# bjing2016/mdgen

Hardware: AMD Instinct MI355X
Metric: sampled MD frames/sec (higher is better)
Workload: dtype bf16

## Files before the change

mdgen_amd/build.py:

```python
from __future__ import annotations

import argparse
import concurrent.futures as cf
import os
import shutil
import subprocess

HERE = os.path.dirname(os.path.abspath(__file__))
CSRC = os.path.join(HERE, "csrc")
OBJ = os.path.join(HERE, "build")
LIB = os.path.join(HERE, "libmdgen_amd.so")
SOURCES = ["api.hip", "k_gemm.hip", "k_rows.hip", "k_flash.hip", "k_small.hip", "k_se3.hip", "k_fp32.hip", "k_optim.hip", "k_fp32_bwd.hip", "k_attn16.hip", "k_wide16.hip", "k_ode.hip"]
HEADERS = ["common.h", "dev.h", "panel.h", "rows.h", "linear.h", "kernels.h", "train.inc", "ode.inc", os.path.join("..", "..", "include", "mdgen_amd.h")]
FLAGS = ["--offload-arch=gfx950", "-O3", "-std=c++17", "-fPIC", "-fno-gpu-rdc", "-fno-slp-vectorize", "-Wall",
         "-Wno-unused-function", "-Wno-pass-failed"]
EXTRA = {"k_flash.hip": ["-fno-honor-nans"]}


def flags_for(src: str):
    return FLAGS + EXTRA.get(os.path.basename(src), [])


def hipcc() -> str:
    for c in (os.environ.get("HIPCC"), shutil.which("hipcc"), "/opt/rocm/bin/hipcc"):
        if c and os.path.exists(c):
            return c
    raise RuntimeError("hipcc not found (set HIPCC)")


_MFMA_RE = None


def check_isa(cc: str, src: str) -> None:
    import re
    import tempfile
    with tempfile.TemporaryDirectory() as td:
        out = os.path.join(td, "k.s")
        r = subprocess.run([cc] + [f for f in flags_for(src) if f not in ("-fPIC",)] + ["-S", "--cuda-device-only", src, "-o", out],
                           capture_output=True, text=True)
        if r.returncode != 0:
            raise RuntimeError("ISA check failed to compile " + src + "\n" + r.stderr)
        pat = re.compile(r"v_mfma_\w+ ([va])\[(\d+):(\d+)\], ([va])\[(\d+):(\d+)\], ([va])\[(\d+):(\d+)\], (.*)$")
        n = 0
        own_m0 = os.path.basename(src) in ("k_rows.hip", "k_wide16.hip")
        in_asm = False
        for line in open(out):
            if own_m0:
                if "#ASMSTART" in line:
                    in_asm = True
                elif "#ASMEND" in line:
                    in_asm = False
                elif not in_asm and re.search(r"\bm0\b", line.split(";")[0]):
                    raise RuntimeError(f"{os.path.basename(src)}: compiler-generated M0 access: {line.strip()}")
            if re.search(r"\bv_pk_(mul|add|fma)_f32\b", line):
                raise RuntimeError(f"{os.path.basename(src)}: packed fp32 VALU op emitted: {line.strip()}")
            m = pat.search(line)
            if not m:
                continue
            n += 1
            g = m.groups()
            dc, ac, bc = g[0], g[3], g[6]
            d0, d1, a0, a1, b0, b1 = int(g[1]), int(g[2]), int(g[4]), int(g[5]), int(g[7]), int(g[8])
            if (ac == dc and not (a1 < d0 or a0 > d1)) or (bc == dc and not (b1 < d0 or b0 > d1)):
                raise RuntimeError(f"{os.path.basename(src)}: MFMA destination overlaps a source operand: {line.strip()}")
    return n


def _stale(target, deps):
    if not os.path.exists(target):
        return True
    t = os.path.getmtime(target)
    return any(os.path.getmtime(d) > t for d in deps)


def build(force: bool = False, jobs: int = 8, verbose: bool = True) -> str:
    os.makedirs(OBJ, exist_ok=True)
    cc = hipcc()
    hdrs = [os.path.join(CSRC, h) for h in HEADERS]
    todo = []
    objs = []
    for src in SOURCES:
        s = os.path.join(CSRC, src)
        o = os.path.join(OBJ, src.replace(".hip", ".o"))
        objs.append(o)
        if force or _stale(o, [s] + hdrs):
            todo.append((s, o))

    def compile_one(so):
        s, o = so
        cmd = [cc] + flags_for(s) + ["-c", s, "-o", o]
        r = subprocess.run(cmd, capture_output=True, text=True)
        if r.returncode != 0:
            raise RuntimeError("hipcc failed: " + " ".join(cmd) + "\n" + r.stdout + r.stderr)
        if os.path.basename(s).startswith("k_"):
            try:
                check_isa(cc, s)
            except Exception:
                if os.path.exists(o):
                    os.remove(o)
                raise
        return s, r.stderr

    if todo:
        with cf.ThreadPoolExecutor(max_workers=jobs) as ex:
            for s, err in ex.map(compile_one, todo):
                if verbose:
                    print("compiled", os.path.basename(s))
                    if err.strip():
                        print(err.strip())
    if force or todo or _stale(LIB, objs):
        cmd = [cc, "--offload-arch=gfx950", "-shared", "-fPIC", "-o", LIB] + objs
        r = subprocess.run(cmd, capture_output=True, text=True)
        if r.returncode != 0:
            raise RuntimeError("link failed: " + " ".join(cmd) + "\n" + r.stdout + r.stderr)
        if verbose:
            print("linked", LIB)
    return LIB


if __name__ == "__main__":
    ap = argparse.ArgumentParser()
    ap.add_argument("--force", action="store_true")
    ap.add_argument("-j", type=int, default=8)
    a = ap.parse_args()
    print(build(force=a.force, jobs=a.j))
```

mdgen_amd/csrc/k_flash.hip:

```cpp
#include "kernels.h"
#include "panel.h"
#include <type_traits>

namespace mdg {

__device__ __forceinline__ bf16x8 frag16(const unsigned char* p) { return *reinterpret_cast<const bf16x8*>(p); }

__device__ __forceinline__ bf16x8 frag8(const unsigned char* p) {
    const u32x2 v = *reinterpret_cast<const u32x2*>(p);
    const u32x4 w = u32x4{v[0], v[1], 0u, 0u};
    return __builtin_bit_cast(bf16x8, w);
}

struct KTile {
    u32x4 k0;
    u32x4 k1;
};
struct VTile {
    u32x4 v0;
    u32x4 v1;
};
struct QTile {
    bf16x8 q0, q1;
};
struct PTile {
    u32x4 p0, p1;
};

struct Half {
    f32x16 o;
    float m;
    unsigned long long unanch;
};

__device__ __forceinline__ float half_max(float x) {
    const auto r = __builtin_amdgcn_permlane32_swap(__float_as_uint(x), __float_as_uint(x), false, false);
    return fmaxf(__uint_as_float(r[0]), __uint_as_float(r[1]));
}

__device__ __forceinline__ float round_bf16(float x) { return __uint_as_float(pack_bf16(x, 0.f) << 16); }

__device__ __forceinline__ float set_shift(QTile& q, float m, int hh) {
    const float hi = round_bf16(m), lo = round_bf16(m - hi);
    if (hh == 0) {
        q.q1[4] = (__bf16)(-hi);
        q.q1[5] = (__bf16)(-lo);
    }
    return hi + lo;
}

constexpr float kAnchor = 63.f;

__device__ __forceinline__ void mask_scores(f32x16& s, uint32_t vm, int hh) {
    uint32_t vmh;
    asm volatile("v_lshrrev_b32 %0, %1, %2" : "=v"(vmh) : "v"(4 * hh), "s"(vm));
#pragma unroll
    for (int r = 0; r < 16; ++r) {
        const bool ok = (vmh >> ((r & 3) + 8 * (r >> 2))) & 1u;
        s[r] = ok ? s[r] : -1e30f;
    }
}

__device__ __forceinline__ f32x16 scores(const KTile& k, const QTile& q) {
    const bf16x8 k0 = __builtin_bit_cast(bf16x8, k.k0), k1 = __builtin_bit_cast(bf16x8, k.k1);
    const f32x16 zero = {0.f, 0.f, 0.f, 0.f, 0.f, 0.f, 0.f, 0.f, 0.f, 0.f, 0.f, 0.f, 0.f, 0.f, 0.f, 0.f};
    f32x16 s = __builtin_amdgcn_mfma_f32_32x32x16_bf16(k0, q.q0, zero, 0, 0, 0);
    s = __builtin_amdgcn_mfma_f32_32x32x16_bf16(k1, q.q1, s, 0, 0, 0);
    asm volatile("" :: "v"(k0), "v"(k1), "v"(q.q0), "v"(q.q1));
    return s;
}

__device__ __forceinline__ void block(const KTile& kn, const QTile& qn, f32x16& n,
                                      const VTile& vp, const PTile& pp, f32x16& od,
                                      const f32x16& s, PTile& pc) {
    const bf16x8 k0 = __builtin_bit_cast(bf16x8, kn.k0), k1 = __builtin_bit_cast(bf16x8, kn.k1);
    const f32x16 zero = {0.f, 0.f, 0.f, 0.f, 0.f, 0.f, 0.f, 0.f, 0.f, 0.f, 0.f, 0.f, 0.f, 0.f, 0.f, 0.f};
    od = __builtin_amdgcn_mfma_f32_32x32x16_bf16(__builtin_bit_cast(bf16x8, vp.v0), __builtin_bit_cast(bf16x8, pp.p0), od, 0, 0, 0);
    n = __builtin_amdgcn_mfma_f32_32x32x16_bf16(k0, qn.q0, zero, 0, 0, 0);
    od = __builtin_amdgcn_mfma_f32_32x32x16_bf16(__builtin_bit_cast(bf16x8, vp.v1), __builtin_bit_cast(bf16x8, pp.p1), od, 0, 0, 0);
    n = __builtin_amdgcn_mfma_f32_32x32x16_bf16(k1, qn.q1, n, 0, 0, 0);
    float e[16];
#pragma unroll
    for (int j = 0; j < 16; ++j) e[j] = __builtin_amdgcn_exp2f(s[j]);
#pragma unroll
    for (int j = 0; j < 4; ++j) {
#ifdef MDGEN_DEV_FLASH_TRUNC
        pc.p0[j] = __builtin_amdgcn_perm(__float_as_uint(e[2 * j + 1]), __float_as_uint(e[2 * j]), 0x07060302u);
        pc.p1[j] = __builtin_amdgcn_perm(__float_as_uint(e[9 + 2 * j]), __float_as_uint(e[8 + 2 * j]), 0x07060302u);
#else
        pc.p0[j] = pack_bf16(e[2 * j], e[2 * j + 1]);
        pc.p1[j] = pack_bf16(e[8 + 2 * j], e[9 + 2 * j]);
#endif
    }
#pragma unroll
    for (int g = 0; g < 4; ++g) {
        __builtin_amdgcn_sched_group_barrier(0x008, 1, 0);
        __builtin_amdgcn_sched_group_barrier(0x402, 6, 0);
    }
    asm volatile("" : "+v"(pc.p0), "+v"(pc.p1) : "v"(k0), "v"(k1), "v"(qn.q0), "v"(qn.q1));
}

constexpr float kDefer = 8.f;

__device__ __forceinline__ void softmax_stats(Half& st, f32x16& s, QTile& q, uint32_t vm, int hh) {
    if (vm != 0xffffffffu) mask_scores(s, vm, hh);
    float t = fmaxf(s[0], s[1]);
#pragma unroll
    for (int r = 2; r < 16; r += 2) t = fmaxf(fmaxf(t, s[r]), s[r + 1]);
    t = half_max(t);
    if ((__builtin_amdgcn_ballot_w64(t > kDefer) | st.unanch) != 0) {
        const bool fin = t > -1e29f;
        const bool un = (st.unanch >> lane_id()) & 1ull;
        const bool mv = (t > kDefer) | (un & fin & (t < -kDefer));
        st.unanch &= ~__builtin_amdgcn_ballot_w64(fin);
        const float r = set_shift(q, mv ? st.m + t : st.m, hh);
        const float e = r - st.m;
        st.m = r;
        const float a = __builtin_amdgcn_exp2f(fminf(-e, 0.f));
#pragma unroll
        for (int i = 0; i < 16; ++i) {
            st.o[i] *= a;
            s[i] -= e;
        }
    }
}

#ifdef MDGEN_DEV_FLASH_STAMPS
__device__ unsigned long long g_flash_stamps[32768 * 16];
extern "C" int mdgen_dev_flash_stamps(void* host, size_t bytes) {
    return (int)hipMemcpyFromSymbol(host, HIP_SYMBOL(g_flash_stamps), bytes);
}
#define FLASH_STAMP(slot, v)                                                                          \
    if (lane == 0 && (long)blockIdx.x * 4 + w < 32768) g_flash_stamps[((long)blockIdx.x * 4 + w) * 16 + (slot)] = (v)
__device__ unsigned long long g_fproj_stamps[8192 * 16];
extern "C" int mdgen_dev_fproj_stamps(void* host, size_t bytes) {
    return (int)hipMemcpyFromSymbol(host, HIP_SYMBOL(g_fproj_stamps), bytes);
}
#define FPROJ_STAMP(slot, v)                                                                          \
    if (lane_id() == 0 && (long)blockIdx.x * 4 + w < 8192) g_fproj_stamps[((long)blockIdx.x * 4 + w) * 16 + (slot)] = (v)
#define FLASH_STAMP_ROW(w, hg) ((w) + 4096 * (hg))
#else
#define FLASH_STAMP(slot, v)
#define FPROJ_STAMP(slot, v)
#define FLASH_STAMP_ROW(w, hg) (w)
#endif

template <int N, class F>
__device__ __forceinline__ void static_for(F&& f) {
    if constexpr (N > 0) {
        static_for<N - 1>(f);
        f(std::integral_constant<int, N - 1>{});
    }
}

struct FlashStoreGlobal {
    __bf16* obuf;
    AxisMap ax;
    int seq, head;
    __device__ __forceinline__ void row(int, int pos, u32x2 a, u32x2 b, u32x2 c) const {
        u32x2* d = reinterpret_cast<u32x2*>(obuf + ax.token(seq, pos) * kC + head * kDH + (lane_id() >> 5) * 12);
        d[0] = a;
        d[1] = b;
        d[2] = c;
    }
    __device__ __forceinline__ void pad(int, int) const {}
};

template <int NQ>
struct FlashPre {
    QTile q[NQ];
    u32x4 kb0;
    u32x2 kb1;
    f32x4 bvl[3];
    KTile k0t;
    uint32_t vmw;
};

__device__ __forceinline__ void* flash_uniform_ptr(const unsigned char* q_) {
    const unsigned long long a = (unsigned long long)q_;
    const unsigned lo = __builtin_amdgcn_readfirstlane((unsigned)a), hi = __builtin_amdgcn_readfirstlane((unsigned)(a >> 32));
    return (void*)(((unsigned long long)hi << 32) | lo);
}

template <int NQ>
__device__ __forceinline__ void flash_prefetch(const FlashParams p, const int seq, const int head, const int qc, FlashPre<NQ>& pre) {
    const int lane = lane_id(), hh = lane >> 5;
    const int len = p.ax.len, nt = p.ax.ntile();
    const long ftile = (long)(seq * kH + head) * nt;
    const unsigned char* qb = p.qf + ftile * kFragQ;
    const int qt0 = NQ * qc;
#pragma unroll
    for (int j = 0; j < NQ; ++j) {
        const int qt = (qt0 + j) * 32 < len ? qt0 + j : qt0;
        pre.q[j].q0 = frag16(qb + (long)qt * kFragQ + lane * 16);
        pre.q[j].q1 = frag8(qb + (long)qt * kFragQ + 1024 + lane * 8);
    }
    const bool bias_alone = (len & 31) == 0 && len >= 32;
    const unsigned char* kb = p.kf + (ftile + (bias_alone ? (len >> 5) : 0)) * kFragK + hh * 32 * 16;
    pre.kb0 = *reinterpret_cast<const u32x4*>(kb);
    pre.kb1 = *reinterpret_cast<const u32x2*>(kb + 1024);
    const f32x4* bv = reinterpret_cast<const f32x4*>(p.bias_v + head * kDH + hh * 12);
    pre.bvl[0] = bv[0];
    pre.bvl[1] = bv[1];
    pre.bvl[2] = bv[2];
    const __amdgpu_buffer_rsrc_t krs = __builtin_amdgcn_make_buffer_rsrc(flash_uniform_ptr(p.kf + ftile * kFragK), 0, 0x7fffffff, 0x00020000);
    pre.k0t.k0 = __builtin_amdgcn_raw_buffer_load_b128(krs, lane * 16, 0, 0);
    pre.k0t.k1 = __builtin_amdgcn_raw_buffer_load_b128(krs, lane * 16 + 1024, 0, 0);
    pre.vmw = (p.vmask + (long)seq * p.vmask_stride)[lane];
}

template <int NQ, class Store>
__device__ __forceinline__ void flash_job(const FlashParams p, const int seq, const int head, const int qc, const int w,
                                          const FlashPre<NQ> pre, const Store store) {
    const int lane = lane_id(), hh = lane >> 5, ql = lane & 31;
    FLASH_STAMP(0, __builtin_amdgcn_s_memtime());
    FLASH_STAMP(4, __builtin_amdgcn_s_memrealtime());
    const int len = p.ax.len, nt = p.ax.ntile();
    const long ftile = (long)(seq * kH + head) * nt;
    const int qt0 = NQ * qc;
    QTile q[NQ];
    bool qvalid[NQ];
#pragma unroll
    for (int j = 0; j < NQ; ++j) {
        qvalid[j] = (qt0 + j) * 32 < len;
        q[j] = pre.q[j];
    }
    const bool bias_alone = (len & 31) == 0 && len >= 32;
    const u32x4 kb0 = pre.kb0;
    const u32x2 kb1 = pre.kb1;
    const f32x4 bvl[3] = {pre.bvl[0], pre.bvl[1], pre.bvl[2]};

    const __amdgpu_buffer_rsrc_t krs = __builtin_amdgcn_make_buffer_rsrc(flash_uniform_ptr(p.kf + ftile * kFragK), 0, 0x7fffffff, 0x00020000);
    const __amdgpu_buffer_rsrc_t vrs = __builtin_amdgcn_make_buffer_rsrc(flash_uniform_ptr(p.vf + ftile * kFragV), 0, 0x7fffffff, 0x00020000);
    const int koff = lane * 16;
    const int voff = ql <= kDH ? hh * 400 + ql * 16 : (int)0x80000000;
    auto issue_k = [&](KTile& t, int kt) __attribute__((always_inline)) {
        t.k0 = __builtin_amdgcn_raw_buffer_load_b128(krs, koff, kt * kFragK, 0);
        t.k1 = __builtin_amdgcn_raw_buffer_load_b128(krs, koff + 1024, kt * kFragK, 0);
    };
    auto issue_v = [&](VTile& t, int kt) __attribute__((always_inline)) {
        t.v0 = __builtin_amdgcn_raw_buffer_load_b128(vrs, voff, kt * kFragV, 0);
        t.v1 = __builtin_amdgcn_raw_buffer_load_b128(vrs, voff + 800, kt * kFragV, 0);
    };
    const KTile k0t = pre.k0t;
    const uint32_t* vmrow = p.vmask + (long)seq * p.vmask_stride;
    uint32_t vmw = pre.vmw;

    Half h[NQ];
    f32x16 s[2];
    PTile pt[2];
    KTile kx, ky;
    VTile vx, vy;
    int rot = 0, nrun = 1;
    auto phys = [&](int i) __attribute__((always_inline)) {
        const int t = i + rot;
        return t >= nrun ? t - nrun : t;
    };
    auto tile = [&](auto robust, int ti, KTile& kc, KTile& kn, VTile& vc, VTile& vprev) __attribute__((always_inline)) {
        constexpr bool kRobust = decltype(robust)::value;
        const int t = kRobust ? ti : phys(ti);
        const uint32_t vm = __builtin_amdgcn_readlane(vmw, t & 63);
        static_for<NQ>([&](auto J) __attribute__((always_inline)) {
            constexpr int j = decltype(J)::value;
            if constexpr (kRobust) softmax_stats(h[j], s[j & 1], q[j], vm, hh);
            else if (vm != 0xffffffffu) mask_scores(s[j & 1], vm, hh);
            __builtin_amdgcn_sched_barrier(0);
            if constexpr (j == 0) block(kc, q[1], s[1], vprev, pt[(NQ - 1) & 1], h[NQ - 1].o, s[0], pt[0]);
            else if constexpr (j < NQ - 1) block(kc, q[j + 1], s[(j + 1) & 1], vc, pt[(j - 1) & 1], h[j - 1].o, s[j & 1], pt[j & 1]);
            else block(kn, q[0], s[0], vc, pt[(j - 1) & 1], h[j - 1].o, s[j & 1], pt[j & 1]);
            __builtin_amdgcn_sched_barrier(0);
#ifndef MDGEN_DEV_FLASH_NOLOAD
            if constexpr (j == 0) issue_v(vprev, kRobust ? ti + 1 : phys(ti + 1));
            if constexpr (j == NQ - 2) issue_k(kc, kRobust ? ti + 2 : phys(ti + 2));
            if constexpr (j == 0 || j == NQ - 2) __builtin_amdgcn_sched_barrier(0);
#endif
        });
    };
    auto run = [&](auto robust, const int nt, const int rot_) __attribute__((always_inline)) {
        rot = rot_;
        nrun = nt;
#pragma unroll
        for (int j = 0; j < NQ; ++j)
#pragma unroll
            for (int r = 0; r < 16; ++r) h[j].o[r] = opaque_zero();
        pt[(NQ - 1) & 1].p0 = pt[(NQ - 1) & 1].p1 = u32x4{0u, 0u, 0u, 0u};
        if (nt > 64) vmw = vmrow[lane];
        issue_k(kx, phys(0));
        issue_v(vy, phys(0));
        issue_k(ky, phys(1));
        issue_v(vx, phys(0));
        __builtin_amdgcn_sched_barrier(0);
        s[0] = scores(kx, q[0]);
        int t = 0;
        for (; t + 1 < nt; t += 2) {
            if ((t & 63) == 0 && t) vmw = vmrow[t + lane];
            tile(robust, t, kx, ky, vx, vy);
            tile(robust, t + 1, ky, kx, vy, vx);
        }
        const bf16x8 lp0 = __builtin_bit_cast(bf16x8, pt[(NQ - 1) & 1].p0), lp1 = __builtin_bit_cast(bf16x8, pt[(NQ - 1) & 1].p1);
        if (t < nt) {
            if ((t & 63) == 0 && t) vmw = vmrow[t + lane];
            tile(robust, t, kx, ky, vx, vy);
            h[NQ - 1].o = __builtin_amdgcn_mfma_f32_32x32x16_bf16(__builtin_bit_cast(bf16x8, vx.v0), __builtin_bit_cast(bf16x8, pt[(NQ - 1) & 1].p0), h[NQ - 1].o, 0, 0, 0);
            h[NQ - 1].o = __builtin_amdgcn_mfma_f32_32x32x16_bf16(__builtin_bit_cast(bf16x8, vx.v1), __builtin_bit_cast(bf16x8, pt[(NQ - 1) & 1].p1), h[NQ - 1].o, 0, 0, 0);
        } else {
            h[NQ - 1].o = __builtin_amdgcn_mfma_f32_32x32x16_bf16(__builtin_bit_cast(bf16x8, vy.v0), lp0, h[NQ - 1].o, 0, 0, 0);
            h[NQ - 1].o = __builtin_amdgcn_mfma_f32_32x32x16_bf16(__builtin_bit_cast(bf16x8, vy.v1), lp1, h[NQ - 1].o, 0, 0, 0);
        }
    };

    if (nt <= 64 && !p.force_robust) {
        const uint32_t want = lane == (len >> 5) ? 1u << (len & 31) : 0u;
        const bool only_bias = __builtin_amdgcn_ballot_w64(lane < nt && vmw != want) == 0;
        if (only_bias) {
            const f32x4 b0 = bvl[0], b1 = bvl[1], b2 = bvl[2];
            const u32x2 d0 = {pack_bf16(b0[0], b0[1]), pack_bf16(b0[2], b0[3])}, d1 = {pack_bf16(b1[0], b1[1]), pack_bf16(b1[2], b1[3])},
                        d2 = {pack_bf16(b2[0], b2[1]), pack_bf16(b2[2], b2[3])};
#pragma unroll
            for (int j = 0; j < NQ; ++j) {
                const int pos = (qt0 + j) * 32 + ql;
                if (qvalid[j] && pos < len) store.row(j, pos, d0, d1, d2);
                else store.pad(j, pos);
            }
            return;
        }
    }
    const int nt_fast = bias_alone ? nt - 1 : nt;
    float sbias[NQ], vbias[12];
    if (bias_alone) {
        const f32x4 b0 = bvl[0], b1 = bvl[1], b2 = bvl[2];
#pragma unroll
        for (int i = 0; i < 4; ++i) {
            vbias[i] = round_bf16(b0[i]);
            vbias[4 + i] = round_bf16(b1[i]);
            vbias[8 + i] = round_bf16(b2[i]);
        }
#pragma unroll
        for (int j = 0; j < NQ; ++j) {
            const u32x4 qa = __builtin_bit_cast(u32x4, q[j].q0);
            const u32x4 qb_ = __builtin_bit_cast(u32x4, q[j].q1);
            float d = 0.f;
#pragma unroll
            for (int i = 0; i < 4; ++i) d += bf16_lo(qa[i]) * bf16_lo(kb0[i]) + bf16_hi(qa[i]) * bf16_hi(kb0[i]);
#pragma unroll
            for (int i = 0; i < 2; ++i) d += bf16_lo(qb_[i]) * bf16_lo(kb1[i]) + bf16_hi(qb_[i]) * bf16_hi(kb1[i]);
            sbias[j] = d + __shfl_xor(d, 32, 64);
        }
    }
    bool robust_needed = p.force_robust != 0;
    {
        const uint32_t vm0 = __builtin_amdgcn_readlane(vmw, 0);
#pragma unroll
        for (int j = 0; j < NQ; ++j) {
            f32x16 s0 = scores(k0t, q[j]);
            if (vm0 != 0xffffffffu) mask_scores(s0, vm0, hh);
            float t0 = fmaxf(s0[0], s0[1]);
#pragma unroll
            for (int r = 2; r < 16; r += 2) t0 = fmaxf(fmaxf(t0, s0[r]), s0[r + 1]);
            t0 = half_max(t0);
            robust_needed |= __builtin_amdgcn_ballot_w64(!(t0 > -1e29f)) != 0;
            h[j].m = set_shift(q[j], t0 + kAnchor, hh);
        }
    }
    FLASH_STAMP(1, __builtin_amdgcn_s_memtime());
    FLASH_STAMP(6, (unsigned long long)robust_needed);
    FLASH_STAMP(8, (unsigned long long)__float_as_uint(h[0].m));
    if (!robust_needed) {
        run(std::false_type{}, nt_fast, (p.rotate && nt_fast > 2 && nt <= 64) ? (qc * nt_fast) / ((len + 32 * NQ - 1) / (32 * NQ)) : 0);
        if (bias_alone) {
#pragma unroll
            for (int j = 0; j < NQ; ++j) {
                const float pb = __builtin_amdgcn_exp2f(sbias[j] - h[j].m);
#pragma unroll
                for (int r = 0; r < 12; ++r) h[j].o[r] += pb * vbias[r];
                if (hh == 0) h[j].o[12] += pb;
            }
        }
        FLASH_STAMP(2, __builtin_amdgcn_s_memtime());
        bool bad = false;
#pragma unroll
        for (int j = 0; j < NQ; ++j) {
            const uint32_t lj = __float_as_uint(h[j].o[12]);
            bad |= (lj & 0x7f800000u) == 0x7f800000u;
            bad |= hh == 0 && (lj & 0x7f800000u) == 0u;
#pragma unroll
            for (int i = 0; i < 16; ++i) bad |= (__float_as_uint(h[j].o[i]) & 0x7f800000u) == 0x7f800000u;
        }
        FLASH_STAMP(9, (unsigned long long)__builtin_amdgcn_ballot_w64(bad));
        robust_needed = __builtin_amdgcn_ballot_w64(bad) != 0;
#ifdef MDGEN_DEV_FLASH_NOFALLBACK
        robust_needed = false;
#endif
    }
    if (robust_needed) {
#pragma unroll
        for (int j = 0; j < NQ; ++j) {
            h[j].m = 0.f;
            h[j].unanch = ~0ull;
            set_shift(q[j], 0.f, hh);
        }
        run(std::true_type{}, nt, 0);
    }
    FLASH_STAMP(3, __builtin_amdgcn_s_memtime());
    FLASH_STAMP(11, (unsigned long long)__float_as_uint(h[0].m));
#ifdef MDGEN_DEV_FLASH_STAMPS
    if (lane == 0 && (long)blockIdx.x * 4 + w < 32768) g_flash_stamps[((long)blockIdx.x * 4 + w) * 16 + 6] |= (unsigned long long)robust_needed << 1;
#endif
#pragma unroll
    for (int j = 0; j < NQ; ++j) {
        const float l = __shfl(h[j].o[12], ql, 64);
        const int pos = (qt0 + j) * 32 + ql;
        if (qvalid[j] && pos < len) {
            const float inv = 1.0f / l;
            const f32x16 o = h[j].o;
            store.row(j, pos, u32x2{pack_bf16(o[0] * inv, o[1] * inv), pack_bf16(o[2] * inv, o[3] * inv)},
                      u32x2{pack_bf16(o[4] * inv, o[5] * inv), pack_bf16(o[6] * inv, o[7] * inv)},
                      u32x2{pack_bf16(o[8] * inv, o[9] * inv), pack_bf16(o[10] * inv, o[11] * inv)});
        } else {
            store.pad(j, pos);
        }
    }
    FLASH_STAMP(5, __builtin_amdgcn_s_memrealtime());
}

template <int NQ>
__global__ __launch_bounds__(256, NQ == 2 ? 3 : 2) void k_flash(const FlashParams p) {
    const int w = __builtin_amdgcn_readfirstlane(wave_id());
    const int nqc = (p.ax.len + 32 * NQ - 1) / (32 * NQ);
    const int xcd = blockIdx.x & 7, rest = blockIdx.x >> 3;
    const int qc = rest % nqc, pair = (rest / nqc) * 8 + xcd;
    const int seq = pair >> 2, hg = pair & 3;
    if (seq >= p.ax.nseq) return;
    const int head = hg * 4 + w;
    FlashPre<NQ> pre;
    flash_prefetch<NQ>(p, seq, head, qc, pre);
    flash_job<NQ>(p, seq, head, qc, w, pre, FlashStoreGlobal{p.obuf, p.ax, seq, head});
}

typedef __attribute__((address_space(3))) unsigned char lds_byte;
struct FlashStorePanel {
    lds_byte* panel;
    int head;
    __device__ __forceinline__ void put(int j, u32x2 a, u32x2 b, u32x2 c) const {
        const int lane = lane_id(), row = 32 * j + (lane & 31), byte = head * 48 + (lane >> 5) * 24;
        typedef __attribute__((address_space(3))) u32x2 lds_u32x2;
        *reinterpret_cast<lds_u32x2*>(panel + panel_off(row, byte, kC * 2)) = a;
        *reinterpret_cast<lds_u32x2*>(panel + panel_off(row, byte + 8, kC * 2)) = b;
        *reinterpret_cast<lds_u32x2*>(panel + panel_off(row, byte + 16, kC * 2)) = c;
    }
    __device__ __forceinline__ void row(int j, int, u32x2 a, u32x2 b, u32x2 c) const { put(j, a, b, c); }
    __device__ __forceinline__ void pad(int j, int) const { put(j, u32x2{0u, 0u}, u32x2{0u, 0u}, u32x2{0u, 0u}); }
};

__global__ __launch_bounds__(256, 2) void k_flash_proj(const FlashProjParams p) {
    constexpr int NQ = 2;
    static_assert(32 * NQ == kPanel, "one workgroup = one 64-row panel");
    __shared__ __attribute__((aligned(16))) unsigned char smem[sizeof(PanelRows) + kPanel * kC * 2];
    PanelRows* pr = reinterpret_cast<PanelRows*>(smem);
    unsigned char* panel = smem + sizeof(PanelRows);
    const int w = __builtin_amdgcn_readfirstlane(wave_id());
    const int nqc = (p.f.ax.len + kPanel - 1) / kPanel;
    const int xcd = blockIdx.x & 7, rest = blockIdx.x >> 3;
    const int qc = rest % nqc, seq = (rest / nqc) * 8 + xcd;
    if (seq >= p.f.ax.nseq) return;
    FPROJ_STAMP(0, __builtin_amdgcn_s_memtime());
    FPROJ_STAMP(8, __builtin_amdgcn_s_memrealtime());
    FPROJ_STAMP(10, (unsigned long long)__builtin_amdgcn_s_getreg((31 << 11) | 4));
    setup_rows_axis(pr, p.f.ax, seq, qc * kPanel, p.mm);
    FlashPre<NQ> cur;
    flash_prefetch<NQ>(p.f, seq, w, qc, cur);
#pragma unroll 1
    for (int hg = 0; hg < 4; ++hg) {
        FlashPre<NQ> nxt;
        flash_prefetch<NQ>(p.f, seq, 4 * (hg < 3 ? hg + 1 : 3) + w, qc, nxt);
        __builtin_amdgcn_sched_barrier(0);
        flash_job<NQ>(p.f, seq, 4 * hg + w, qc, FLASH_STAMP_ROW(w, hg), cur, FlashStorePanel{(lds_byte*)panel, 4 * hg + w});
        cur = nxt;
        FPROJ_STAMP(1 + hg, __builtin_amdgcn_s_memtime());
    }
    __syncthreads();
    FPROJ_STAMP(5, __builtin_amdgcn_s_memtime());
    const int lane = lane_id();
    f32x16 acc[6];
#ifndef MDGEN_DEV_FLASH_NOEARLY
    EpiPre<8> ep;
    epi_rmw_request<8>(0, 0, pr, 96 * w, p.h, ep);
    __builtin_amdgcn_sched_barrier(0);
#endif
    zero_acc<6>(acc);
    wave_gemm<2, 3, 24, false>(panel, kC * 2, 0, 0, p.wo + (size_t)(3 * w) * 24 * 64 + lane, 24 * 64, acc);
    FPROJ_STAMP(6, __builtin_amdgcn_s_memtime());
    __syncthreads();
#ifndef MDGEN_DEV_FLASH_NOEARLY
    epilogue_gate_residual_lds_pre<3>(acc, pr, reinterpret_cast<float*>(panel) + w * (32 * 96), 96 * w, p.bo, p.mm, p.gate_chunk, true,
                                      p.h, ep);
#else
    epilogue_gate_residual_lds<3>(acc, pr, reinterpret_cast<float*>(panel) + w * (32 * 96), 96 * w, p.bo, p.mm, p.gate_chunk, true,
                                  p.h);
#endif
    FPROJ_STAMP(7, __builtin_amdgcn_s_memtime());
    FPROJ_STAMP(9, __builtin_amdgcn_s_memrealtime());
}

__global__ __launch_bounds__(512, 1) void k_flash_proj8(const FlashProjParams p) {
    constexpr int NQ = 4, kRows = 32 * NQ;
    __shared__ __attribute__((aligned(16))) unsigned char smem[2 * sizeof(PanelRows) + kRows * kC * 2];
    PanelRows* pr = reinterpret_cast<PanelRows*>(smem);
// ... 77 lines not shown
```

mdgen_amd/csrc/k_gemm.hip:

```cpp
#include "kernels.h"
#include "panel.h"

namespace mdg {

constexpr int kRowB = kC * 2;
constexpr int kPanelBytes = kPanel * kRowB;

template <bool ROPE, int TT = 2>
__device__ __forceinline__ void epilogue_heads_T(const f32x16* acc , const PanelRows* pr, int w,
                                                 const float* __restrict__ bias_perm, const float* __restrict__ rope,
                                                 bool small, int pos0, int len, int seq, int ntile, int tile0,
                                                 unsigned char* __restrict__ frag, __bf16* __restrict__ small_dst,
                                                 int which) {
    const int lane = lane_id(), hh = lane >> 5, tk = lane & 31;
    f32x4 bq[4][3];
    {
        const f32x4* bp = reinterpret_cast<const f32x4*>(bias_perm + (w * 2 + hh) * 48);
#pragma unroll
        for (int hd = 0; hd < 4; ++hd)
#pragma unroll
            for (int c = 0; c < 3; ++c) bq[hd][c] = bp[hd * 3 + c];
    }
    int tokv[TT], posv[TT];
    f32x4 rq[TT][4];
#pragma unroll
    for (int tt = 0; tt < TT; ++tt) {
        const int row = tt * 32 + tk;
        tokv[tt] = pr->tok[row];
        int pos = small ? (tokv[tt] >= 0 ? tokv[tt] % len : 0) : pos0 + row;
        if (pos > len) pos = len;
        posv[tt] = pos;
        if (ROPE) {
            const f32x4* rc = reinterpret_cast<const f32x4*>(rope + (long)pos * kRopeRow + 16 * hh);
#pragma unroll
            for (int i = 0; i < 4; ++i) rq[tt][i] = rc[i];
        }
    }
#pragma unroll
    for (int tt = 0; tt < TT; ++tt) {
        const int token = tokv[tt];
        const bool valid = token >= 0;
        float cs[6], sn[6];
        if (ROPE) {
#pragma unroll
            for (int p = 0; p < 6; ++p) {
                cs[p] = rq[tt][p >> 2][p & 3];
                sn[p] = rq[tt][2 + (p >> 2)][p & 3];
            }
        }
        const int tile = tile0 + tt;
#pragma unroll
        for (int hd = 0; hd < 4; ++hd) {
            float e[12];
#pragma unroll
            for (int c = 0; c < 3; ++c) {
                const int ap = 3 * hd + c, ft = ap >> 2, a = ap & 3;
#pragma unroll
                for (int b = 0; b < 4; ++b) e[4 * c + b] = acc[ft * TT + tt][4 * a + b] + bq[hd][c][b];
            }
            if (ROPE) {
#pragma unroll
                for (int p = 0; p < 6; ++p) {
                    const float x1 = e[2 * p], x2 = e[2 * p + 1];
                    e[2 * p] = x1 * cs[p] - x2 * sn[p];
                    e[2 * p + 1] = x2 * cs[p] + x1 * sn[p];
                }
            }
            uint32_t u[6];
#pragma unroll
            for (int i = 0; i < 6; ++i) u[i] = pack_bf16(e[2 * i], e[2 * i + 1]);
            const int head = 4 * w + hd;
            if (small) {
                if (valid) {
                    u32x2* d = reinterpret_cast<u32x2*>(small_dst + (long)token * (3 * kC) + which * kC + head * kDH + hh * 12);
                    d[0] = u32x2{u[0], u[1]};
                    d[1] = u32x2{u[2], u[3]};
                    d[2] = u32x2{u[4], u[5]};
                }
            } else if (tile < ntile) {
                if (which == 1) {
                    unsigned char* base = frag + ((long)(seq * kH + head) * ntile + tile) * kFragK;
                    *reinterpret_cast<u32x4*>(base + lane * 16) = u32x4{u[0], u[1], u[2], u[3]};
                    *reinterpret_cast<u32x4*>(base + 1024 + lane * 16) = u32x4{u[4], u[5], 0x3f803f80u, 0u};
                } else {
                    unsigned char* base = frag + ((long)(seq * kH + head) * ntile + tile) * kFragQ;
                    *reinterpret_cast<u32x4*>(base + lane * 16) = u32x4{u[0], u[1], u[2], u[3]};
                    *reinterpret_cast<u32x2*>(base + 1024 + lane * 8) = u32x2{u[4], u[5]};
                }
            }
        }
    }
}

template <int TT = 2>
__device__ __forceinline__ void epilogue_v_flash(const f32x16* acc , int w,
                                                 const float* __restrict__ bias_perm, int seq, int ntile, int tile0,
                                                 unsigned char* __restrict__ vf) {
    const int lane = lane_id(), hh = lane >> 5, n = lane & 31;
#pragma unroll
    for (int j = 0; j < 3; ++j) {
        const int col = 32 * j + n;
        const int hd = col / kDH, d = col - hd * kDH;
        const float b = bias_perm[w * 96 + col];
        const int head = 4 * w + hd;
#pragma unroll
        for (int tt = 0; tt < TT; ++tt) {
            const int tile = tile0 + tt;
            if (tile < ntile) {
                unsigned char* base = vf + ((long)(seq * kH + head) * ntile + tile) * kFragV + hh * 400 + d * 16;
                const f32x16 a = acc[tt * 3 + j];
                *reinterpret_cast<u32x4*>(base) = u32x4{pack_bf16(a[0] + b, a[1] + b), pack_bf16(a[2] + b, a[3] + b),
                                                         pack_bf16(a[4] + b, a[5] + b), pack_bf16(a[6] + b, a[7] + b)};
                *reinterpret_cast<u32x4*>(base + 800) =
                    u32x4{pack_bf16(a[8] + b, a[9] + b), pack_bf16(a[10] + b, a[11] + b),
                          pack_bf16(a[12] + b, a[13] + b), pack_bf16(a[14] + b, a[15] + b)};
            }
        }
    }
    if (lane < 32) {
        const int hd = lane & 3, tt = (lane >> 2) & 1, h2 = (lane >> 3) & 1, ks = lane >> 4;
        const int tile = tile0 + tt;
        if (tt < TT && tile < ntile)
            *reinterpret_cast<u32x4*>(vf + ((long)(seq * kH + 4 * w + hd) * ntile + tile) * kFragV + ks * 800 + h2 * 400 + kDH * 16) =
                u32x4{0x3f803f80u, 0x3f803f80u, 0x3f803f80u, 0x3f803f80u};
    }
}

__device__ __forceinline__ void write_bias_slots(const QkvParams& p, int seq, int w, bool do_k = true, bool do_v = true, int tpp = 2) {
    const int lane = lane_id();
    const int len = p.ax.len, nt = p.ax.ntile();
    const int kt = len >> 5, sl = len & 31;
    if (kt >= tpp * p.panels_per_seq) {
#pragma unroll
        for (int hd = 0; hd < 4; ++hd) {
            const long ft = (long)(seq * kH + 4 * w + hd) * nt + kt;
            u32x4* kd = reinterpret_cast<u32x4*>(p.kf + ft * kFragK);
            u32x4* vd = reinterpret_cast<u32x4*>(p.vf + ft * kFragV);
            const u32x4 z = {0u, 0u, 0u, 0u}, ones = {0x3f803f80u, 0x3f803f80u, 0x3f803f80u, 0x3f803f80u};
            if (do_k) {
                kd[lane] = z;
                kd[64 + lane] = u32x4{0u, 0u, 0x3f803f80u, 0u};
            }
            const int r0 = lane, r1 = 64 + lane;
            if (do_v) {
                vd[r0] = (r0 % 25) == kDH ? ones : z;
                if (r1 < 100) vd[r1] = (r1 % 25) == kDH ? ones : z;
            }
        }
        __builtin_amdgcn_sched_barrier(0);
    }
    if (do_k && lane < 8) {
        const int hd = lane & 3, hh = lane >> 2, head = 4 * w + hd;
        const float* bk = p.bias_k + head * kDH;
        const float* rc = p.rope + (long)len * kRopeRow + 16 * hh;
        float e[12];
#pragma unroll
        for (int pp = 0; pp < 6; ++pp) {
            const int i = 6 * hh + pp;
            const float x1 = bk[i], x2 = bk[i + 12], c = rc[pp], sn = rc[8 + pp];
            e[2 * pp] = x1 * c - x2 * sn;
            e[2 * pp + 1] = x2 * c + x1 * sn;
        }
        unsigned char* base = p.kf + ((long)(seq * kH + head) * nt + kt) * kFragK;
        *reinterpret_cast<u32x4*>(base + (hh * 32 + sl) * 16) =
            u32x4{pack_bf16(e[0], e[1]), pack_bf16(e[2], e[3]), pack_bf16(e[4], e[5]), pack_bf16(e[6], e[7])};
        *reinterpret_cast<u32x4*>(base + 1024 + (hh * 32 + sl) * 16) =
            u32x4{pack_bf16(e[8], e[9]), pack_bf16(e[10], e[11]), 0x3f803f80u, 0u};
    }
    if (do_v && lane < kDH) {
        const int d = lane;
        const int dpsi = 12 * ((d >> 2) & 1) + 4 * (d >> 3) + (d & 3);
        const int hk = (sl >> 2) & 1, r = (sl & 3) + 4 * (sl >> 3);
#pragma unroll
        for (int hd = 0; hd < 4; ++hd) {
            const int head = 4 * w + hd;
            unsigned char* base = p.vf + ((long)(seq * kH + head) * nt + kt) * kFragV;
            const uint32_t v = pack_bf16(p.bias_v[head * kDH + dpsi], 0.f);
            *reinterpret_cast<uint16_t*>(base + (r >> 3) * 800 + hk * 400 + d * 16 + (r & 7) * 2) = (uint16_t)v;
        }
    }
}

#ifdef MDGEN_DEV_QKV_STAMPS
__device__ unsigned long long g_qkv_stamps[16384 * 8];
extern "C" int mdgen_dev_qkv_stamps(void* host, size_t bytes) {
    return (int)hipMemcpyFromSymbol(host, HIP_SYMBOL(g_qkv_stamps), bytes);
}
#define QKV_STAMP(slot)                                                                                      \
    if (!SMALL && lane_id() == 0 && (long)blockIdx.x * 4 + wave_id() < 16384)                                  \
    g_qkv_stamps[((long)blockIdx.x * 4 + wave_id()) * 8 + (slot)] = __builtin_amdgcn_s_memtime()
__device__ unsigned long long g_attn4_stamps[8192 * 16];
extern "C" int mdgen_dev_attn4_stamps(void* host, size_t bytes) {
    return (int)hipMemcpyFromSymbol(host, HIP_SYMBOL(g_attn4_stamps), bytes);
}
#define ATTN4_STAMP_DECL unsigned long long a4st[11] = {}
#define ATTN4_STAMP(slot)                          \
    a4st[slot] = __builtin_amdgcn_s_memtime();     \
    __builtin_amdgcn_sched_barrier(0)
#define ATTN4_STAMP_FLUSH                                                                                   \
    if (lane_id() == 0 && (long)blockIdx.x * 4 + wave_id() < 8192) {                                          \
        _Pragma("unroll") for (int k = 0; k < 11; ++k)                                                        \
            g_attn4_stamps[((long)blockIdx.x * 4 + wave_id()) * 16 + k] = a4st[k];                            \
    }
#else
#define QKV_STAMP(slot)
#define ATTN4_STAMP_DECL
#define ATTN4_STAMP(slot)
#define ATTN4_STAMP_FLUSH
#endif

template <bool SMALL, bool PRE = false>
__global__ __launch_bounds__(256, 2) void k_ln_qkv(const QkvParams p) {
    __shared__ __attribute__((aligned(16))) unsigned char smem[sizeof(PanelRows) + kPanelBytes];
    PanelRows* pr = reinterpret_cast<PanelRows*>(smem);
    unsigned char* panel = smem + sizeof(PanelRows);
    int seq = 0, pos0 = 0, tile0 = 0;
    if (SMALL) {
        setup_rows_linear(pr, (long)blockIdx.x * kPanel, p.nrows, p.mm);
    } else {
        seq = blockIdx.x / p.panels_per_seq;
        const int pn = blockIdx.x - seq * p.panels_per_seq;
        pos0 = pn * kPanel;
        tile0 = pn * 2;
        setup_rows_axis(pr, p.ax, seq, pos0, p.mm);
        if (wave_id() == 0) {
            const int lane = lane_id(), len = p.ax.len, pos = pos0 + lane;
            const float mv = p.mk.at(p.ax.token(seq, pos < len ? pos : len - 1));
            const unsigned long long bal = __ballot(pos == len || (pos < len && mv != 0.f));
            uint32_t* vm = p.vmask + (long)seq * p.vmask_stride;
            if (lane < 2) vm[tile0 + lane] = (uint32_t)(bal >> (32 * lane));
            if (pn == p.panels_per_seq - 1) {
                const int idx = tile0 + 2 + lane;
                if (idx < p.vmask_stride) vm[idx] = idx == (len >> 5) ? 1u << (len & 31) : 0u;
                if (idx + 64 < p.vmask_stride) vm[idx + 64] = 0u;
            }
        }
    }
    QKV_STAMP(0);
    __syncthreads();
    const int w = __builtin_amdgcn_readfirstlane(wave_id()), lane = lane_id();
    f32x16 acc[6];
    if (PRE) {
        prologue_bf16<kC>(panel, pr, p.obuf);
        __syncthreads();
        zero_acc<6>(acc);
        wave_gemm<2, 3, 24, false>(panel, kRowB, 0, 0, p.wo + (size_t)(3 * w) * 24 * 64 + lane, 24 * 64, acc);
        __syncthreads();
        epilogue_gate_residual_lds<3>(acc, pr, reinterpret_cast<float*>(panel) + w * (32 * 96), 96 * w, p.bo, p.mm, p.gate_chunk,
                                      true, p.h_rw);
        __syncthreads();
    }
    prologue_ln<false>(panel, pr, PRE ? p.h_rw : p.h, p.mm, p.shift_chunk, p.scale_chunk, 1e-6f);
    __syncthreads();
    QKV_STAMP(1);
    const int ntile = p.ax.ntile();
    const int len = p.ax.len;
    zero_acc<6>(acc);
    wave_gemm<2, 3, 24, true>(panel, kRowB, 0, 0, p.wq + (size_t)(3 * w) * 24 * 64 + lane, 24 * 64, acc);
    QKV_STAMP(2);
    epilogue_heads_T<true>(acc, pr, w, p.bq, p.rope, SMALL, pos0, len, seq, ntile, tile0, p.qf, p.qkv_small, 0);
    __builtin_amdgcn_sched_barrier(0);
    QKV_STAMP(3);
    zero_acc<6>(acc);
    wave_gemm<2, 3, 24, true>(panel, kRowB, 0, 0, p.wk + (size_t)(3 * w) * 24 * 64 + lane, 24 * 64, acc);
    QKV_STAMP(4);
    epilogue_heads_T<true>(acc, pr, w, p.bk, p.rope, SMALL, pos0, len, seq, ntile, tile0, p.kf, p.qkv_small, 1);
    __builtin_amdgcn_sched_barrier(0);
    QKV_STAMP(5);
    zero_acc<6>(acc);
    if (SMALL) {
        wave_gemm<2, 3, 24, true>(panel, kRowB, 0, 0, p.wv + (size_t)(3 * w) * 24 * 64 + lane, 24 * 64, acc);
        epilogue_heads_T<false>(acc, pr, w, p.bv, nullptr, true, pos0, len, seq, ntile, tile0, nullptr, p.qkv_small, 2);
    } else {
        wave_gemm<2, 3, 24, false>(panel, kRowB, 0, 0, p.wv + (size_t)(3 * w) * 24 * 64 + lane, 24 * 64, acc);
        QKV_STAMP(6);
        epilogue_v_flash(acc, w, p.bv, seq, ntile, tile0, p.vf);
        if ((int)blockIdx.x - seq * p.panels_per_seq == p.panels_per_seq - 1) {
            __builtin_amdgcn_sched_barrier(0);
            write_bias_slots(p, seq, w);
        }
        QKV_STAMP(7);
    }
}

template <int J>
__device__ __forceinline__ float quad_bcast(float v) {
    return __builtin_bit_cast(float, __builtin_amdgcn_update_dpp(0, __builtin_bit_cast(int, v), J * 0x55, 0xf, 0xf, true));
}
__device__ __forceinline__ float half_sum(float x) {
    const auto r = __builtin_amdgcn_permlane32_swap(__float_as_uint(x), __float_as_uint(x), false, false);
    return __uint_as_float(r[0]) + __uint_as_float(r[1]);
}
template <int TT = 2>
__device__ __forceinline__ void head_values(const f32x16* acc, int tt, int hd, const f32x4 (&bq)[3], float (&e)[12]) {
#pragma unroll
    for (int c = 0; c < 3; ++c) {
        const int ap = 3 * hd + c, ft = ap >> 2, a = ap & 3;
#pragma unroll
        for (int b = 0; b < 4; ++b) e[4 * c + b] = acc[ft * TT + tt][4 * a + b] + bq[c][b];
    }
}
__device__ __forceinline__ void load_head_bias(const float* bias_perm, int w, int hh, f32x4 (&bq)[4][3]) {
    const f32x4* bp = reinterpret_cast<const f32x4*>(bias_perm + (w * 2 + hh) * 48);
#pragma unroll
    for (int hd = 0; hd < 4; ++hd)
#pragma unroll
        for (int c = 0; c < 3; ++c) bq[hd][c] = bp[hd * 3 + c];
}


template <bool SPLIT, bool HALF = false>
__global__ __launch_bounds__(512, 1) void k_ln_qkv8(const QkvParams p) {
    static_assert(!HALF || SPLIT, "32-row workgroups exist in the split form only");
    constexpr int TT = HALF ? 1 : 2, kRows = 32 * TT;
    __shared__ __attribute__((aligned(16))) unsigned char smem[sizeof(PanelRows) + kPanelBytes];
    PanelRows* pr = reinterpret_cast<PanelRows*>(smem);
    unsigned char* panel = smem + sizeof(PanelRows);
    const int blk = SPLIT ? blockIdx.x >> 1 : blockIdx.x, half = SPLIT ? blockIdx.x & 1 : 0;
    const int seq = blk / p.panels_per_seq;
    const int pn = blk - seq * p.panels_per_seq;
// ... 956 lines not shown
```

Measured before the change: 120,000.

## Stop storing constant K-fragment padding; synthesize it in registers in flash attention

The K fragment's second half used to store a constant bf16 1.0 / zero pair per lane in global memory, and every K tile load read 16 bytes for it. Producers now write only the 8 meaningful bytes. The flash kernel loads 8 bytes and fills the constant lanes once with inline asm, so the compiler cannot rematerialise them, and a build check rejects any compiler-generated copy of the constant. Q prefetch also moves to buffer loads. This cuts K write and read traffic and register moves, at the cost of coupling the producer layout to the consumer and relying on the registers staying intact across the loop.

```diff
diff --git a/mdgen_amd/build.py b/mdgen_amd/build.py
--- a/mdgen_amd/build.py
+++ b/mdgen_amd/build.py
@@ -44,14 +44,16 @@
         n = 0
         own_m0 = os.path.basename(src) in ("k_rows.hip", "k_wide16.hip")
         in_asm = False
+        k_const = os.path.basename(src) == "k_flash.hip"
         for line in open(out):
-            if own_m0:
-                if "#ASMSTART" in line:
-                    in_asm = True
-                elif "#ASMEND" in line:
-                    in_asm = False
-                elif not in_asm and re.search(r"\bm0\b", line.split(";")[0]):
-                    raise RuntimeError(f"{os.path.basename(src)}: compiler-generated M0 access: {line.strip()}")
+            if "#ASMSTART" in line:
+                in_asm = True
+            elif "#ASMEND" in line:
+                in_asm = False
+            elif own_m0 and not in_asm and re.search(r"\bm0\b", line.split(";")[0]):
+                raise RuntimeError(f"{os.path.basename(src)}: compiler-generated M0 access: {line.strip()}")
+            elif k_const and not in_asm and "0x3f803f80" in line.split(";")[0]:
+                raise RuntimeError(f"{os.path.basename(src)}: K operand constant re-materialised by the compiler: {line.strip()}")
             if re.search(r"\bv_pk_(mul|add|fma)_f32\b", line):
                 raise RuntimeError(f"{os.path.basename(src)}: packed fp32 VALU op emitted: {line.strip()}")
             m = pat.search(line)
diff --git a/mdgen_amd/csrc/k_flash.hip b/mdgen_amd/csrc/k_flash.hip
--- a/mdgen_amd/csrc/k_flash.hip
+++ b/mdgen_amd/csrc/k_flash.hip
@@ -4,18 +4,15 @@
 
 namespace mdg {
 
-__device__ __forceinline__ bf16x8 frag16(const unsigned char* p) { return *reinterpret_cast<const bf16x8*>(p); }
-
-__device__ __forceinline__ bf16x8 frag8(const unsigned char* p) {
-    const u32x2 v = *reinterpret_cast<const u32x2*>(p);
-    const u32x4 w = u32x4{v[0], v[1], 0u, 0u};
-    return __builtin_bit_cast(bf16x8, w);
-}
-
 struct KTile {
     u32x4 k0;
     u32x4 k1;
 };
+__device__ __forceinline__ u32x4 k_const_half() {
+    u32x4 k = {0u, 0u, 0u, 0u};
+    asm volatile("v_mov_b32 %0, 0x3f803f80\n\tv_mov_b32 %1, 0\n\ts_nop 1" : "=v"(k[2]), "=v"(k[3]));
+    return k;
+}
 struct VTile {
     u32x4 v0;
     u32x4 v1;
@@ -172,7 +169,8 @@
     u32x4 kb0;
     u32x2 kb1;
     f32x4 bvl[3];
-    KTile k0t;
+    u32x4 k0t0;
+    u32x2 k0t1;
     uint32_t vmw;
 };
 
@@ -187,25 +185,26 @@
     const int lane = lane_id(), hh = lane >> 5;
     const int len = p.ax.len, nt = p.ax.ntile();
     const long ftile = (long)(seq * kH + head) * nt;
-    const unsigned char* qb = p.qf + ftile * kFragQ;
+    const __amdgpu_buffer_rsrc_t qrs = __builtin_amdgcn_make_buffer_rsrc(flash_uniform_ptr(p.qf + ftile * kFragQ), 0, 0x7fffffff, 0x00020000);
     const int qt0 = NQ * qc;
 #pragma unroll
     for (int j = 0; j < NQ; ++j) {
         const int qt = (qt0 + j) * 32 < len ? qt0 + j : qt0;
-        pre.q[j].q0 = frag16(qb + (long)qt * kFragQ + lane * 16);
-        pre.q[j].q1 = frag8(qb + (long)qt * kFragQ + 1024 + lane * 8);
+        pre.q[j].q0 = __builtin_bit_cast(bf16x8, __builtin_amdgcn_raw_buffer_load_b128(qrs, lane * 16, qt * kFragQ, 0));
+        const u32x2 v = __builtin_amdgcn_raw_buffer_load_b64(qrs, lane * 8, qt * kFragQ + 1024, 0);
+        pre.q[j].q1 = __builtin_bit_cast(bf16x8, u32x4{v[0], v[1], 0u, 0u});
     }
     const bool bias_alone = (len & 31) == 0 && len >= 32;
-    const unsigned char* kb = p.kf + (ftile + (bias_alone ? (len >> 5) : 0)) * kFragK + hh * 32 * 16;
-    pre.kb0 = *reinterpret_cast<const u32x4*>(kb);
-    pre.kb1 = *reinterpret_cast<const u32x2*>(kb + 1024);
     const f32x4* bv = reinterpret_cast<const f32x4*>(p.bias_v + head * kDH + hh * 12);
     pre.bvl[0] = bv[0];
     pre.bvl[1] = bv[1];
     pre.bvl[2] = bv[2];
     const __amdgpu_buffer_rsrc_t krs = __builtin_amdgcn_make_buffer_rsrc(flash_uniform_ptr(p.kf + ftile * kFragK), 0, 0x7fffffff, 0x00020000);
-    pre.k0t.k0 = __builtin_amdgcn_raw_buffer_load_b128(krs, lane * 16, 0, 0);
-    pre.k0t.k1 = __builtin_amdgcn_raw_buffer_load_b128(krs, lane * 16 + 1024, 0, 0);
+    pre.k0t0 = __builtin_amdgcn_raw_buffer_load_b128(krs, lane * 16, 0, 0);
+    pre.k0t1 = __builtin_amdgcn_raw_buffer_load_b64(krs, lane * 8, 1024, 0);
+    const int kbt = bias_alone ? (len >> 5) * kFragK : 0;
+    pre.kb0 = __builtin_amdgcn_raw_buffer_load_b128(krs, hh * 32 * 16, kbt, 0);
+    pre.kb1 = __builtin_amdgcn_raw_buffer_load_b64(krs, hh * 32 * 8, kbt + 1024, 0);
     pre.vmw = (p.vmask + (long)seq * p.vmask_stride)[lane];
 }
 
@@ -232,17 +231,18 @@
 
     const __amdgpu_buffer_rsrc_t krs = __builtin_amdgcn_make_buffer_rsrc(flash_uniform_ptr(p.kf + ftile * kFragK), 0, 0x7fffffff, 0x00020000);
     const __amdgpu_buffer_rsrc_t vrs = __builtin_amdgcn_make_buffer_rsrc(flash_uniform_ptr(p.vf + ftile * kFragV), 0, 0x7fffffff, 0x00020000);
-    const int koff = lane * 16;
+    const int koff = lane * 16, koff1 = lane * 8;
     const int voff = ql <= kDH ? hh * 400 + ql * 16 : (int)0x80000000;
     auto issue_k = [&](KTile& t, int kt) __attribute__((always_inline)) {
         t.k0 = __builtin_amdgcn_raw_buffer_load_b128(krs, koff, kt * kFragK, 0);
-        t.k1 = __builtin_amdgcn_raw_buffer_load_b128(krs, koff + 1024, kt * kFragK, 0);
+        const u32x2 d = __builtin_amdgcn_raw_buffer_load_b64(krs, koff1, kt * kFragK + 1024, 0);
+        t.k1[0] = d[0];
+        t.k1[1] = d[1];
     };
     auto issue_v = [&](VTile& t, int kt) __attribute__((always_inline)) {
         t.v0 = __builtin_amdgcn_raw_buffer_load_b128(vrs, voff, kt * kFragV, 0);
         t.v1 = __builtin_amdgcn_raw_buffer_load_b128(vrs, voff + 800, kt * kFragV, 0);
     };
-    const KTile k0t = pre.k0t;
     const uint32_t* vmrow = p.vmask + (long)seq * p.vmask_stride;
     uint32_t vmw = pre.vmw;
 
@@ -350,9 +350,14 @@
     bool robust_needed = p.force_robust != 0;
     {
         const uint32_t vm0 = __builtin_amdgcn_readlane(vmw, 0);
+        kx.k1 = k_const_half();
+        ky.k1 = k_const_half();
+        kx.k0 = pre.k0t0;
+        kx.k1[0] = pre.k0t1[0];
+        kx.k1[1] = pre.k0t1[1];
 #pragma unroll
         for (int j = 0; j < NQ; ++j) {
-            f32x16 s0 = scores(k0t, q[j]);
+            f32x16 s0 = scores(kx, q[j]);
             if (vm0 != 0xffffffffu) mask_scores(s0, vm0, hh);
             float t0 = fmaxf(s0[0], s0[1]);
 #pragma unroll
diff --git a/mdgen_amd/csrc/k_gemm.hip b/mdgen_amd/csrc/k_gemm.hip
--- a/mdgen_amd/csrc/k_gemm.hip
+++ b/mdgen_amd/csrc/k_gemm.hip
@@ -78,15 +78,9 @@
                     d[2] = u32x2{u[4], u[5]};
                 }
             } else if (tile < ntile) {
-                if (which == 1) {
-                    unsigned char* base = frag + ((long)(seq * kH + head) * ntile + tile) * kFragK;
-                    *reinterpret_cast<u32x4*>(base + lane * 16) = u32x4{u[0], u[1], u[2], u[3]};
-                    *reinterpret_cast<u32x4*>(base + 1024 + lane * 16) = u32x4{u[4], u[5], 0x3f803f80u, 0u};
-                } else {
-                    unsigned char* base = frag + ((long)(seq * kH + head) * ntile + tile) * kFragQ;
-                    *reinterpret_cast<u32x4*>(base + lane * 16) = u32x4{u[0], u[1], u[2], u[3]};
-                    *reinterpret_cast<u32x2*>(base + 1024 + lane * 8) = u32x2{u[4], u[5]};
-                }
+                unsigned char* base = frag + ((long)(seq * kH + head) * ntile + tile) * (which == 1 ? kFragK : kFragQ);
+                *reinterpret_cast<u32x4*>(base + lane * 16) = u32x4{u[0], u[1], u[2], u[3]};
+                *reinterpret_cast<u32x2*>(base + 1024 + lane * 8) = u32x2{u[4], u[5]};
             }
         }
     }
@@ -139,7 +133,7 @@
             const u32x4 z = {0u, 0u, 0u, 0u}, ones = {0x3f803f80u, 0x3f803f80u, 0x3f803f80u, 0x3f803f80u};
             if (do_k) {
                 kd[lane] = z;
-                kd[64 + lane] = u32x4{0u, 0u, 0x3f803f80u, 0u};
+                if (lane < 32) kd[64 + lane] = z;
             }
             const int r0 = lane, r1 = 64 + lane;
             if (do_v) {
@@ -164,8 +158,7 @@
         unsigned char* base = p.kf + ((long)(seq * kH + head) * nt + kt) * kFragK;
         *reinterpret_cast<u32x4*>(base + (hh * 32 + sl) * 16) =
             u32x4{pack_bf16(e[0], e[1]), pack_bf16(e[2], e[3]), pack_bf16(e[4], e[5]), pack_bf16(e[6], e[7])};
-        *reinterpret_cast<u32x4*>(base + 1024 + (hh * 32 + sl) * 16) =
-            u32x4{pack_bf16(e[8], e[9]), pack_bf16(e[10], e[11]), 0x3f803f80u, 0u};
+        *reinterpret_cast<u32x2*>(base + 1024 + (hh * 32 + sl) * 8) = u32x2{pack_bf16(e[8], e[9]), pack_bf16(e[10], e[11])};
     }
     if (do_v && lane < kDH) {
         const int d = lane;
```

Result: no change. 120,900 (median of 6 runs) (+0.8%).
